# fischer-hub/panGNN

Hardware: AMD Instinct MI355X
Metric: edges/sec in GNN forward+backward (link-pred train step) (higher is better)
Workload: dtype f32

## Files before the change

### pangnn_amd/csrc/linear.hip

```cpp
#include "common.h"

namespace pangnn {

typedef float f32x16 __attribute__((ext_vector_type(16)));

__device__ __forceinline__ constexpr int jrow(int r, int hh) { return (r & 3) + 8 * (r >> 2) + 4 * hh; }

__device__ __forceinline__ void wave_sync_lds() {
  __builtin_amdgcn_fence(__ATOMIC_RELEASE, "wavefront");
  __builtin_amdgcn_wave_barrier();
  __builtin_amdgcn_fence(__ATOMIC_ACQUIRE, "wavefront");
}

__device__ __forceinline__ void pin(int64_t& base, uint32_t& off) { asm volatile("" : "+s"(base), "+v"(off)); }
__device__ __forceinline__ float4 ld_f4(const float* ubase, uint32_t byte_off) {
  typedef float f32x4 __attribute__((ext_vector_type(4)));
  const f32x4 t = __builtin_nontemporal_load(reinterpret_cast<const f32x4*>(reinterpret_cast<const char*>(ubase) + byte_off));
  return make_float4(t[0], t[1], t[2], t[3]);
}
__device__ __forceinline__ void st_f32(float* ubase, uint32_t byte_off, float v) {
  *reinterpret_cast<float*>(reinterpret_cast<char*>(ubase) + byte_off) = v;
}

typedef unsigned short bf16s;
// ... 58 lines not shown
struct RowRegs { typename Elem<T>::raw4 v[32 / (64 / (C / 4))]; };

template <int C, typename T>
__device__ __forceinline__ void load_rows_full(const T* __restrict__ src, int64_t ld, int64_t base, int lane,
                                               RowRegs<C, T>& rg) {
  constexpr int LPR = C / 4;
  constexpr int RPI = 64 / LPR;
  const int c4 = lane % LPR, r0 = lane / LPR;
  uint32_t loff = ((uint32_t)r0 * (uint32_t)ld + 4u * c4) * (uint32_t)sizeof(T);
  pin(base, loff);
#pragma unroll
  for (int i = 0; i < 32 / RPI; ++i) rg.v[i] = Elem<T>::ld4(src + (base + i * RPI) * ld, loff);
}

template <int C, typename T>
__device__ __forceinline__ void load_rows(const T* __restrict__ src, int64_t ld, int64_t n, int64_t base,
                                          int lane, RowRegs<C, T>& rg) {
  constexpr int LPR = C / 4;
  constexpr int RPI = 64 / LPR;
  const int c4 = lane % LPR, r0 = lane / LPR;
  if (base + 32 <= n) {
    load_rows_full<C, T>(src, ld, base, lane, rg);
    return;
  }
#pragma unroll
  for (int i = 0; i < 32 / RPI; ++i) {
    const int row = i * RPI + r0;
    rg.v[i] = Elem<T>::zero4();
    if (base + row < n) rg.v[i] = Elem<T>::ld4_plain(src + (base + row) * ld + 4 * c4);
  }
}

__device__ __forceinline__ float elu1(float v) { return v > 0.f ? v : __expf(v) - 1.f; }
__device__ __forceinline__ float elu1_grad(float v) { return v > 0.f ? 1.f : __expf(v); }
__device__ __forceinline__ float gen_h(float rv, float sv, float a, float c, float b) { return fmaf(rv, a, fmaf(sv, c, b)); }

template <int C, int ACT = 0, typename T = float>
__device__ __forceinline__ void store_rows(const RowRegs<C, T>& rg, int lane, float* tile) {
  constexpr int LPR = C / 4;
  constexpr int RPI = 64 / LPR;
  constexpr int RS = C + 4;
  const int c4 = lane % LPR, r0 = lane / LPR;
#pragma unroll
  for (int i = 0; i < 32 / RPI; ++i) {
    float4 v = Elem<T>::cvt4(rg.v[i]);
    if (ACT == 1) { v.x = elu1(v.x); v.y = elu1(v.y); v.z = elu1(v.z); v.w = elu1(v.w); }
    *reinterpret_cast<float4*>(tile + (i * RPI + r0) * RS + 4 * c4) = v;
  }
}

template <int K, int M>
struct FwdGeo {
  static constexpr int KS = K + 4;
  static constexpr int WAVES = (K == 128 && M == 128) ? 3 : 4;
};

template <int K, int M>
__device__ __forceinline__ void tile_product(const float* Xt, const float* Wl, int r, int hh, f32x16 (&acc)[M / 32]) {
  constexpr int KS = K + 4;
#pragma unroll
  for (int b = 0; b < M / 32; ++b)
#pragma unroll
    for (int i = 0; i < 16; ++i) acc[b][i] = 0.f;
  const float* xa = Xt + r * KS + 4 * (K / 8) * hh;
  const float* wb = Wl + r * KS + 4 * (K / 8) * hh;
  float4 a = *reinterpret_cast<const float4*>(xa);
  float4 bw[M / 32];
#pragma unroll
  for (int b = 0; b < M / 32; ++b) bw[b] = *reinterpret_cast<const float4*>(wb + 32 * b * KS);
#pragma unroll
  for (int i = 0; i < K / 8; ++i) {
    float4 an = a, bn[M / 32];
#pragma unroll
    for (int b = 0; b < M / 32; ++b) bn[b] = bw[b];
    if (i + 1 < K / 8) {
      an = *reinterpret_cast<const float4*>(xa + 4 * (i + 1));
#pragma unroll
      for (int b = 0; b < M / 32; ++b) bn[b] = *reinterpret_cast<const float4*>(wb + 32 * b * KS + 4 * (i + 1));
    }
    __builtin_amdgcn_sched_barrier(0);
#pragma unroll
    for (int b = 0; b < M / 32; ++b) {
      acc[b] = __builtin_amdgcn_mfma_f32_32x32x2f32(a.x, bw[b].x, acc[b], 0, 0, 0);
      acc[b] = __builtin_amdgcn_mfma_f32_32x32x2f32(a.y, bw[b].y, acc[b], 0, 0, 0);
      acc[b] = __builtin_amdgcn_mfma_f32_32x32x2f32(a.z, bw[b].z, acc[b], 0, 0, 0);
      acc[b] = __builtin_amdgcn_mfma_f32_32x32x2f32(a.w, bw[b].w, acc[b], 0, 0, 0);
    }
    __builtin_amdgcn_sched_barrier(0);
    a = an;
#pragma unroll
    for (int b = 0; b < M / 32; ++b) bw[b] = bn[b];
  }
}

typedef __bf16 bf16x8 __attribute__((ext_vector_type(8)));
typedef unsigned int u32x4v __attribute__((ext_vector_type(4)));
struct Split3 { bf16x8 hi, mid, lo; };
__device__ __forceinline__ Split3 split8(const float4& f0, const float4& f1) {
  const float f[8] = {f0.x, f0.y, f0.z, f0.w, f1.x, f1.y, f1.z, f1.w};
  u32x4v hi, mid, lo;
#pragma unroll
  for (int q = 0; q < 4; ++q) {
    const uint32_t a = __builtin_bit_cast(uint32_t, f[2 * q]), b = __builtin_bit_cast(uint32_t, f[2 * q + 1]);
    hi[q] = __builtin_amdgcn_perm(b, a, 0x07060302u);
    const float ra = f[2 * q] - __builtin_bit_cast(float, a & 0xffff0000u);
    const float rb = f[2 * q + 1] - __builtin_bit_cast(float, b & 0xffff0000u);
    const uint32_t ua = __builtin_bit_cast(uint32_t, ra), ub = __builtin_bit_cast(uint32_t, rb);
    mid[q] = __builtin_amdgcn_perm(ub, ua, 0x07060302u);
    const float sa = ra - __builtin_bit_cast(float, ua & 0xffff0000u);
    const float sb = rb - __builtin_bit_cast(float, ub & 0xffff0000u);
    lo[q] = __builtin_amdgcn_perm(__builtin_bit_cast(uint32_t, sb), __builtin_bit_cast(uint32_t, sa), 0x07060302u);
  }
  Split3 r;
  r.hi = __builtin_bit_cast(bf16x8, hi);
  r.mid = __builtin_bit_cast(bf16x8, mid);
  r.lo = __builtin_bit_cast(bf16x8, lo);
  return r;
}

template <int K, int M>
struct WImg {
  static constexpr int WS = K + 8;
  static constexpr bool X3 = (3 * M * WS * 2 + FwdGeo<K, M>::WAVES * 32 * (K + 4) * 4 <= 156 * 1024);
  static constexpr int FLOATS = X3 ? (3 * M * WS + 1) / 2 : M * (K + 4);
};

template <int K, int M>
__device__ __forceinline__ void stage_w(const float* __restrict__ w, int sm, int sk, float* Wl, int n_threads) {
  if constexpr (WImg<K, M>::X3) {
    constexpr int WS = WImg<K, M>::WS, IMG = M * WS;
    unsigned short* W3 = reinterpret_cast<unsigned short*>(Wl);
#pragma unroll 8
    for (int i = threadIdx.x; i < M * K; i += n_threads) {
      const int m = sk == 1 ? i / K : i % M, k = sk == 1 ? i % K : i / M;
      const float v = w[m * sm + k * sk];
      const uint32_t a = __builtin_bit_cast(uint32_t, v);
      const float r1 = v - __builtin_bit_cast(float, a & 0xffff0000u);
      const uint32_t b = __builtin_bit_cast(uint32_t, r1);
      const float r2 = r1 - __builtin_bit_cast(float, b & 0xffff0000u);
      W3[m * WS + k] = (unsigned short)(a >> 16);
      W3[IMG + m * WS + k] = (unsigned short)(b >> 16);
      W3[2 * IMG + m * WS + k] = (unsigned short)(__builtin_bit_cast(uint32_t, r2) >> 16);
    }
  } else {
    constexpr int KS = K + 4;
#pragma unroll 8
    for (int i = threadIdx.x; i < M * K; i += n_threads) {
      const int m = sk == 1 ? i / K : i % M, k = sk == 1 ? i % K : i / M;
      Wl[m * KS + k] = w[m * sm + k * sk];
    }
  }
}

template <int K, int M>
__device__ __forceinline__ void tile_product_x3(const float* Xt, const float* Wl, int r, int hh, f32x16 (&acc)[M / 32]) {
  constexpr int KS = K + 4, WS = WImg<K, M>::WS, IMG = M * WS;
#pragma unroll
  for (int b = 0; b < M / 32; ++b)
#pragma unroll
    for (int i = 0; i < 16; ++i) acc[b][i] = 0.f;
  const float* xa = Xt + r * KS + 8 * hh;
  const unsigned short* wb = reinterpret_cast<const unsigned short*>(Wl) + r * WS + 8 * hh;
  float4 x0 = *reinterpret_cast<const float4*>(xa), x1 = *reinterpret_cast<const float4*>(xa + 4);
  constexpr bool DB = (M / 32) <= 2;
  bf16x8 wf[DB ? 2 : 1][M / 32][3];
  if constexpr (DB) {
#pragma unroll
    for (int b = 0; b < M / 32; ++b)
#pragma unroll
      for (int t = 0; t < 3; ++t) wf[0][b][t] = *reinterpret_cast<const bf16x8*>(wb + 32 * b * WS + t * IMG);
  }
#pragma unroll
  for (int i = 0; i < K / 16; ++i) {
    if constexpr (!DB) {
#pragma unroll
      for (int b = 0; b < M / 32; ++b)
#pragma unroll
        for (int t = 0; t < 3; ++t) wf[0][b][t] = *reinterpret_cast<const bf16x8*>(wb + 32 * b * WS + 16 * i + t * IMG);
    }
    const Split3 a = split8(x0, x1);
    if (i + 1 < K / 16) {
      x0 = *reinterpret_cast<const float4*>(xa + 16 * (i + 1));
      x1 = *reinterpret_cast<const float4*>(xa + 16 * (i + 1) + 4);
      if constexpr (DB) {
#pragma unroll
        for (int b = 0; b < M / 32; ++b)
#pragma unroll
          for (int t = 0; t < 3; ++t)
            wf[(i + 1) & 1][b][t] = *reinterpret_cast<const bf16x8*>(wb + 32 * b * WS + 16 * (i + 1) + t * IMG);
      }
    }
#define PG_X3(AT, WT)                                                                                     \
    _Pragma("unroll") for (int b = 0; b < M / 32; ++b)                                                    \
      acc[b] = __builtin_amdgcn_mfma_f32_32x32x16_bf16(a.AT, wf[DB ? (i & 1) : 0][b][WT], acc[b], 0, 0, 0);
    PG_X3(lo, 0) PG_X3(hi, 2) PG_X3(mid, 1) PG_X3(mid, 0) PG_X3(hi, 1) PG_X3(hi, 0)
#undef PG_X3
  }
}

template <int K, int M>
__device__ __forceinline__ void tile_mult(const float* Xt, const float* Wl, int r, int hh, f32x16 (&acc)[M / 32]) {
  if constexpr (WImg<K, M>::X3) tile_product_x3<K, M>(Xt, Wl, r, hh, acc);
  else tile_product<K, M>(Xt, Wl, r, hh, acc);
}

template <int K, int M, int ACT, bool GATE, typename TX = float, typename TY = float, typename TG = float>
__global__ __launch_bounds__((FwdGeo<K, M>::WAVES * 64)) void linear_fwd_kernel(const TX* __restrict__ x, int64_t ldx,
                                                         const float* __restrict__ w, int w_sm, int w_sk,
                                                         const float* __restrict__ bias,
                                                         TY* __restrict__ y, int64_t ldy, int64_t n,
                                                         int64_t n_tiles, const TG* __restrict__ gate,
                                                         int64_t ldgate) {
  constexpr int KS = K + 4;
  constexpr int WAVES = FwdGeo<K, M>::WAVES;
  constexpr int WF = (WImg<K, M>::FLOATS + 3) & ~3;
  __shared__ __attribute__((aligned(16))) float lds[WF + WAVES * 32 * KS];
  float* Wl = lds;
  const int wave = __builtin_amdgcn_readfirstlane(threadIdx.x >> 6), lane = threadIdx.x & 63;
  float* Xt = lds + WF + wave * (32 * KS);
  stage_w<K, M>(w, w_sm, w_sk, Wl, WAVES * 64);
  __syncthreads();
  const int r = lane & 31, hh = lane >> 5;
  const int64_t stride = (int64_t)gridDim.x * WAVES;
  const int64_t n_full = n / 32;
  int64_t tile = (int64_t)blockIdx.x * WAVES + wave;
  float bv[M / 32];
#pragma unroll
  for (int b = 0; b < M / 32; ++b) bv[b] = bias ? bias[r + 32 * b] : 0.f;
  f32x16 acc[M / 32];
  RowRegs<K, TX> rg;
  if (tile < n_full) {
    const int64_t last = n_full - 1;
    load_rows_full<K, TX>(x, ldx, tile * 32, lane, rg);
    store_rows<K, ACT, TX>(rg, lane, Xt);
    load_rows_full<K, TX>(x, ldx, (tile + stride < last ? tile + stride : last) * 32, lane, rg);
    wave_sync_lds();
    for (; tile < n_full; tile += stride) {
      float gv[GATE ? M / 32 : 1][16];
      if (GATE) {
        uint32_t goff = (4u * hh * (uint32_t)ldgate + r) * (uint32_t)sizeof(TG);
        int64_t gbase = tile * 32;
        pin(gbase, goff);
#pragma unroll
        for (int i = 0; i < 16; ++i) {
          const TG* gr = gate + (gbase + (i & 3) + 8 * (i >> 2)) * ldgate;
#pragma unroll
          for (int b = 0; b < M / 32; ++b) gv[b][i] = Elem<TG>::ld1(gr + 32 * b, goff);
        }
      }
      tile_mult<K, M>(Xt, Wl, r, hh, acc);
      uint32_t loff = (4u * hh * (uint32_t)ldy + r) * (uint32_t)sizeof(TY);
      int64_t sbase = tile * 32;
      pin(sbase, loff);
#pragma unroll
      for (int i = 0; i < 16; ++i) {
        TY* yr = y + (sbase + (i & 3) + 8 * (i >> 2)) * ldy;
#pragma unroll
        for (int b = 0; b < M / 32; ++b) {
          float v = acc[b][i] + bv[b];
          if (GATE) v *= elu1_grad(gv[b][i]);
          Elem<TY>::st1(yr + 32 * b, loff, v);
        }
      }
      store_rows<K, ACT, TX>(rg, lane, Xt);
      const int64_t nxt = tile + 2 * stride;
      load_rows_full<K, TX>(x, ldx, (nxt < last ? nxt : last) * 32, lane, rg);
      wave_sync_lds();
    }
  }
  if (tile == n_full && n_full < n_tiles) {
    const int64_t base = n_full * 32;
    load_rows<K, TX>(x, ldx, n, base, lane, rg);
    wave_sync_lds();
    store_rows<K, ACT, TX>(rg, lane, Xt);
    wave_sync_lds();
    tile_mult<K, M>(Xt, Wl, r, hh, acc);
#pragma unroll
    for (int b = 0; b < M / 32; ++b)
#pragma unroll
      for (int i = 0; i < 16; ++i) {
        const int64_t row = base + jrow(i, hh);
        if (row < n) {
          float v = acc[b][i] + bv[b];
          if (GATE) v *= elu1_grad(Elem<TG>::ld1(gate + row * ldgate + r + 32 * b, 0u));
          Elem<TY>::st1(y + row * ldy + r + 32 * b, 0u, v);
        }
      }
  }
}

template <int K, int M, int ACT = 0>
__device__ __forceinline__ void wgrad_tile(const float* Xt, const float* Gt, int r, int hh, f32x16 (&acc)[M / 32][K / 32],
                                           float (&gbp)[M / 32]) {
  constexpr int KS = K + 4, MS = M + 4;
#pragma unroll
  for (int j = 0; j < 2; ++j) {
    const int row0 = 16 * j + 8 * hh;
    Split3 ga[M / 32], xb[K / 32];
#pragma unroll
    for (int a = 0; a < M / 32; ++a) {
      float f[8];
#pragma unroll
      for (int q = 0; q < 8; ++q) { f[q] = Gt[(row0 + q) * MS + r + 32 * a]; gbp[a] += f[q]; }
      ga[a] = split8(make_float4(f[0], f[1], f[2], f[3]), make_float4(f[4], f[5], f[6], f[7]));
    }
#pragma unroll
    for (int b = 0; b < K / 32; ++b) {
      float f[8];
#pragma unroll
      for (int q = 0; q < 8; ++q) {
        f[q] = Xt[(row0 + q) * KS + r + 32 * b];
        if (ACT == 1) f[q] = elu1(f[q]);
      }
      xb[b] = split8(make_float4(f[0], f[1], f[2], f[3]), make_float4(f[4], f[5], f[6], f[7]));
    }
#define PG_W3(GT, XT)                                                                                     \
    _Pragma("unroll") for (int a = 0; a < M / 32; ++a)                                                    \
    _Pragma("unroll") for (int b = 0; b < K / 32; ++b)                                                    \
      acc[a][b] = __builtin_amdgcn_mfma_f32_32x32x16_bf16(ga[a].GT, xb[b].XT, acc[a][b], 0, 0, 0);
    PG_W3(lo, hi) PG_W3(hi, lo) PG_W3(mid, mid) PG_W3(mid, hi) PG_W3(hi, mid) PG_W3(hi, hi)
#undef PG_W3
  }
}

template <int K, int M>
__device__ __forceinline__ void gen_wgrad_tile_x3(const float* Gt, const float* rs, const float (&ca)[K / 32],
                                                  const float (&cc)[K / 32], const float (&cb)[K / 32], int r, int hh,
                                                  f32x16 (&acc)[M / 32][K / 32], float (&gbp)[M / 32]) {
  constexpr int MS = M + 4;
#pragma unroll
  for (int j = 0; j < 2; ++j) {
    const int row0 = 16 * j + 8 * hh;
    const float4 R0 = *reinterpret_cast<const float4*>(rs + row0), R1 = *reinterpret_cast<const float4*>(rs + row0 + 4);
    const float4 S0 = *reinterpret_cast<const float4*>(rs + 32 + row0), S1 = *reinterpret_cast<const float4*>(rs + 32 + row0 + 4);
    const float rr[8] = {R0.x, R0.y, R0.z, R0.w, R1.x, R1.y, R1.z, R1.w};
    const float ss[8] = {S0.x, S0.y, S0.z, S0.w, S1.x, S1.y, S1.z, S1.w};
    Split3 ga[M / 32], xb[K / 32];
#pragma unroll
    for (int a = 0; a < M / 32; ++a) {
      float f[8];
#pragma unroll
      for (int q = 0; q < 8; ++q) { f[q] = Gt[(row0 + q) * MS + r + 32 * a]; gbp[a] += f[q]; }
      ga[a] = split8(make_float4(f[0], f[1], f[2], f[3]), make_float4(f[4], f[5], f[6], f[7]));
    }
#pragma unroll
    for (int b = 0; b < K / 32; ++b) {
      float f[8];
#pragma unroll
      for (int q = 0; q < 8; ++q) f[q] = elu1(gen_h(rr[q], ss[q], ca[b], cc[b], cb[b]));
      xb[b] = split8(make_float4(f[0], f[1], f[2], f[3]), make_float4(f[4], f[5], f[6], f[7]));
    }
#define PG_W3(GT, XT)                                                                                     \
    _Pragma("unroll") for (int a = 0; a < M / 32; ++a)                                                    \
    _Pragma("unroll") for (int b = 0; b < K / 32; ++b)                                                    \
      acc[a][b] = __builtin_amdgcn_mfma_f32_32x32x16_bf16(ga[a].GT, xb[b].XT, acc[a][b], 0, 0, 0);
    PG_W3(lo, hi) PG_W3(hi, lo) PG_W3(mid, mid) PG_W3(mid, hi) PG_W3(hi, mid) PG_W3(hi, hi)
#undef PG_W3
  }
}

template <int K, int M>
struct WgradGeo {
  static constexpr int SLAB = M * K + M;
};

template <int K, int M, int LDS_F>
__device__ __forceinline__ void wgrad_finish(const f32x16 (&acc)[M / 32][K / 32], const float (&gbp)[M / 32], float* lds,
                                             float* __restrict__ slab, int wave, int lane) {
  constexpr int NA = (M / 32) * (K / 32) * 16, NV = NA + M / 32;
  static_assert(2 * NV * 64 <= LDS_F, "tree buffers of the wgrad finish");
  const int r = lane & 31, hh = lane >> 5;
  float val[NV];
#pragma unroll
  for (int a = 0; a < M / 32; ++a) {
#pragma unroll
    for (int b = 0; b < K / 32; ++b)
#pragma unroll
      for (int i = 0; i < 16; ++i) val[(a * (K / 32) + b) * 16 + i] = acc[a][b][i];
    val[NA + a] = gbp[a];
  }
  __syncthreads();
#pragma unroll
  for (int d = 1; d < 4; d <<= 1) {
    const bool writer = (wave & (2 * d - 1)) == d, reader = (wave & (2 * d - 1)) == 0;
    float* mine = lds + (size_t)(d == 1 ? (wave >> 1) : 0) * (NV * 64) + lane;
    if (writer) {
#pragma unroll
      for (int v = 0; v < NV; ++v) mine[v * 64] = val[v];
    }
    __syncthreads();
    if (reader) {
#pragma unroll
      for (int v = 0; v < NV; ++v) val[v] += mine[v * 64];
    }
    __syncthreads();
  }
  if (wave == 0) {
#pragma unroll
    for (int a = 0; a < M / 32; ++a) {
#pragma unroll
      for (int b = 0; b < K / 32; ++b)
#pragma unroll
        for (int i = 0; i < 16; ++i) lds[(32 * a + jrow(i, hh)) * K + r + 32 * b] = val[(a * (K / 32) + b) * 16 + i];
      if (hh == 0) lds[M * K + r + 32 * a] = val[NA + a];
    }
  }
  __syncthreads();
  for (int i = threadIdx.x; i < M * K + M; i += 256) slab[i] = lds[i];
}

template <int K, int M, int ACT, typename TG = float, typename TX = float>
__global__ __launch_bounds__(256) void linear_wgrad_kernel(const TG* __restrict__ g, int64_t ldg,
                                                           const TX* __restrict__ x, int64_t ldx,
                                                           int64_t n, int64_t n_tiles,
                                                           float* __restrict__ slabs) {
  constexpr int KS = K + 4, MS = M + 4;
  constexpr int PER_WAVE = 32 * KS + 32 * MS;
  constexpr int SLAB = WgradGeo<K, M>::SLAB;
  constexpr int LDS_F = (4 * PER_WAVE > SLAB) ? 4 * PER_WAVE : SLAB;
  __shared__ __attribute__((aligned(16))) float lds[LDS_F];
  const int wave = __builtin_amdgcn_readfirstlane(threadIdx.x >> 6), lane = threadIdx.x & 63;
  float* Xt = lds + wave * PER_WAVE;
  float* Gt = Xt + 32 * KS;
  const int r = lane & 31, hh = lane >> 5;
  f32x16 acc[M / 32][K / 32];
  float gbp[M / 32];
#pragma unroll
  for (int a = 0; a < M / 32; ++a) {
    gbp[a] = 0.f;
#pragma unroll
    for (int b = 0; b < K / 32; ++b)
#pragma unroll
      for (int i = 0; i < 16; ++i) acc[a][b][i] = 0.f;
  }
  const int64_t stride = (int64_t)gridDim.x * 4;
  int64_t tile = (int64_t)blockIdx.x * 4 + wave;
  RowRegs<K, TX> rx;
  RowRegs<M, TG> rgm;
  load_rows<K, TX>(x, ldx, n, tile * 32, lane, rx);
  load_rows<M, TG>(g, ldg, n, tile * 32, lane, rgm);
  for (; tile < n_tiles; tile += stride) {
    store_rows<K, ACT, TX>(rx, lane, Xt);
    store_rows<M, 0, TG>(rgm, lane, Gt);
    load_rows<K, TX>(x, ldx, n, (tile + stride) * 32, lane, rx);
    load_rows<M, TG>(g, ldg, n, (tile + stride) * 32, lane, rgm);
    wave_sync_lds();
    wgrad_tile<K, M>(Xt, Gt, r, hh, acc, gbp);
    wave_sync_lds();
  }
#pragma unroll
  for (int a = 0; a < M / 32; ++a) gbp[a] += __shfl_xor(gbp[a], 32);
  wgrad_finish<K, M, LDS_F>(acc, gbp, lds, slabs + (int64_t)blockIdx.x * SLAB, wave, lane);
}

__global__ __launch_bounds__(kSumThreads) void slab_reduce_kernel(const float* __restrict__ slabs, int n_slabs,
                                                                  int slab_len, int split,
                                                                  float* __restrict__ out0,
                                                                  float* __restrict__ out1) {
  const int i = blockIdx.x * kWave + (threadIdx.x & (kWave - 1));
  const float s = ordered_parts_sum(slabs, n_slabs, slab_len, i, slab_len);
  if (threadIdx.x >= kWave || i >= slab_len) return;
  if (i < split) out0[i] = s;
  else if (out1) out1[i - split] = s;
}

static int num_cus() {
  int dev = 0, v = 0;
  if (hipGetDevice(&dev) == hipSuccess &&
      hipDeviceGetAttribute(&v, hipDeviceAttributeMultiprocessorCount, dev) == hipSuccess && v > 0)
    return v;
  return 256;
}

template <int K, int M, typename TX, typename TY, typename TG>
static int launch_fwd_t(const void* x, int64_t ldx, const float* w, int w_trans, const float* bias, void* y, int64_t ldy,
                        int64_t n, int in_act, const void* gate, int64_t ldgate, hipStream_t s) {
  const int w_sm = w_trans ? 1 : K, w_sk = w_trans ? M : 1;
  constexpr int WAVES = FwdGeo<K, M>::WAVES;
  const int64_t n_tiles = (n + 31) / 32;
  int64_t grid = (n_tiles + WAVES - 1) / WAVES;
  const int64_t cap = (int64_t)num_cus();
  if (grid > cap) grid = cap;
  const dim3 g((unsigned)grid), b(WAVES * 64);
  const TX* xp = static_cast<const TX*>(x);
  TY* yp = static_cast<TY*>(y);
  const TG* gp = static_cast<const TG*>(gate);
  if (gate)
    hipLaunchKernelGGL((linear_fwd_kernel<K, M, 0, true, TX, TY, TG>), g, b, 0, s, xp, ldx, w, w_sm, w_sk, bias, yp, ldy, n, n_tiles, gp, ldgate);
  else if (in_act)
    hipLaunchKernelGGL((linear_fwd_kernel<K, M, 1, false, TX, TY, float>), g, b, 0, s, xp, ldx, w, w_sm, w_sk, bias, yp, ldy, n, n_tiles,
                       static_cast<const float*>(nullptr), ldgate);
  else
    hipLaunchKernelGGL((linear_fwd_kernel<K, M, 0, false, TX, TY, float>), g, b, 0, s, xp, ldx, w, w_sm, w_sk, bias, yp, ldy, n, n_tiles,
                       static_cast<const float*>(nullptr), ldgate);
  PG_CHECK_LAUNCH("pangnn_linear_fwd");
  return 0;
}

template <int K, int M, typename H>
static int launch_fwd(const void* x, int x16, int64_t ldx, const float* w, int w_trans, const float* bias, void* y,
                      int y16, int64_t ldy, int64_t n, int in_act, const void* gate, int gate16, int64_t ldgate,
                      hipStream_t s) {
#define PG_FWD(TX, TY, TG) return launch_fwd_t<K, M, TX, TY, TG>(x, ldx, w, w_trans, bias, y, ldy, n, in_act, gate, ldgate, s)
  if (gate) {
    if (gate16) { if (x16) PG_FWD(H, H, H); PG_FWD(float, H, H); }
    if (x16) PG_FWD(H, float, float);
    PG_FWD(float, float, float);
  }
  if (x16) { if (y16) PG_FWD(H, H, float); PG_FWD(H, float, float); }
  if (y16) PG_FWD(float, H, float);
// ... 394 lines not shown
      x0.z = elu1(gen_h(rv, sv, a0.z, c0.z, b0.z)); x0.w = elu1(gen_h(rv, sv, a0.w, c0.w, b0.w));
      x1.x = elu1(gen_h(rv, sv, a1.x, c1.x, b1.x)); x1.y = elu1(gen_h(rv, sv, a1.y, c1.y, b1.y));
      x1.z = elu1(gen_h(rv, sv, a1.z, c1.z, b1.z)); x1.w = elu1(gen_h(rv, sv, a1.w, c1.w, b1.w));
      const Split3 a = split8(x0, x1);
#define PG_X3(AT, WT)                                                                                     \
      _Pragma("unroll") for (int b = 0; b < M / 32; ++b)                                                  \
        acc[b] = __builtin_amdgcn_mfma_f32_32x32x16_bf16(a.AT, wf[b][WT], acc[b], 0, 0, 0);
      PG_X3(lo, 0) PG_X3(hi, 2) PG_X3(mid, 1) PG_X3(mid, 0) PG_X3(hi, 1) PG_X3(hi, 0)
#undef PG_X3
    }
    if (tile * 32 + 32 <= n) {
      uint32_t loff = (4u * hh * (uint32_t)ldy + r) * (uint32_t)sizeof(float);
      int64_t sbase = tile * 32;
      pin(sbase, loff);
#pragma unroll
      for (int i = 0; i < 16; ++i) {
        float* yr = y + (sbase + (i & 3) + 8 * (i >> 2)) * ldy;
#pragma unroll
        for (int b = 0; b < M / 32; ++b) st_f32(yr + 32 * b, loff, acc[b][i] + bv[b]);
      }
    } else {
#pragma unroll
      for (int b = 0; b < M / 32; ++b)
#pragma unroll
        for (int i = 0; i < 16; ++i) {
          const int64_t row = tile * 32 + jrow(i, hh);
          if (row < n) y[row * ldy + r + 32 * b] = acc[b][i] + bv[b];
        }
    }
    rv = rn;
    sv = sn;
  }
}

template <int K, int M>
__global__ __launch_bounds__(256) void gen_linear_wgrad_kernel(const float* __restrict__ g, int64_t ldg,
                                                               const float* __restrict__ rvec, const float* __restrict__ svec,
                                                               const float* __restrict__ w_emb, const float* __restrict__ b_emb,
                                                               const float* __restrict__ w_in, const float* __restrict__ b_in,
                                                               int D, int64_t n, int64_t n_tiles, float* __restrict__ slabs) {
  constexpr int KS = K + 4, MS = M + 4;
  constexpr int PER_WAVE = 32 * KS + 32 * MS;
  constexpr int SLAB = WgradGeo<K, M>::SLAB;
  constexpr int LDS_F = (4 * PER_WAVE > SLAB) ? 4 * PER_WAVE : SLAB;
  __shared__ __attribute__((aligned(16))) float lds[LDS_F];
  __shared__ __attribute__((aligned(16))) float acb[3 * K];
  const int wave = __builtin_amdgcn_readfirstlane(threadIdx.x >> 6), lane = threadIdx.x & 63;
  float* Xt = lds + wave * PER_WAVE;
  float* Gt = Xt + 32 * KS;
  gen_params<K>(w_emb, b_emb, w_in, b_in, D, acb, 256);
  __syncthreads();
  const int r = lane & 31, hh = lane >> 5;
  float ca[K / 32], cc[K / 32], cb[K / 32];
#pragma unroll
  for (int b = 0; b < K / 32; ++b) { ca[b] = acb[r + 32 * b]; cc[b] = acb[K + r + 32 * b]; cb[b] = acb[2 * K + r + 32 * b]; }
  f32x16 acc[M / 32][K / 32];
  float gbp[M / 32];
#pragma unroll
  for (int a = 0; a < M / 32; ++a) {
    gbp[a] = 0.f;
#pragma unroll
    for (int b = 0; b < K / 32; ++b)
#pragma unroll
      for (int i = 0; i < 16; ++i) acc[a][b][i] = 0.f;
  }
  const int64_t stride = (int64_t)gridDim.x * 4;
  int64_t tile = (int64_t)blockIdx.x * 4 + wave;
  RowRegs<M, float> rgm;
  float rsv = gen_load(rvec, svec, n, tile * 32, lane);
  load_rows<M, float>(g, ldg, n, tile * 32, lane, rgm);
  for (; tile < n_tiles; tile += stride) {
    Xt[lane] = rsv;
    store_rows<M, 0, float>(rgm, lane, Gt);
    rsv = gen_load(rvec, svec, n, (tile + stride) * 32, lane);
    load_rows<M, float>(g, ldg, n, (tile + stride) * 32, lane, rgm);
    wave_sync_lds();
    gen_wgrad_tile_x3<K, M>(Gt, Xt, ca, cc, cb, r, hh, acc, gbp);
    wave_sync_lds();
  }
#pragma unroll
  for (int a = 0; a < M / 32; ++a) gbp[a] += __shfl_xor(gbp[a], 32);
  wgrad_finish<K, M, LDS_F>(acc, gbp, lds, slabs + (int64_t)blockIdx.x * SLAB, wave, lane);
}

template <int KG, int H>
__global__ __launch_bounds__((FwdGeo<KG, H>::WAVES * 64)) void gen_linear_dgrad_sums_kernel(
    const float* __restrict__ g, int64_t ldg, const float* __restrict__ w_out, const float* __restrict__ rvec,
    const float* __restrict__ svec, const float* __restrict__ w_emb, const float* __restrict__ b_emb,
    const float* __restrict__ w_in, const float* __restrict__ b_in, int D, int64_t n, int64_t n_tiles,
    float* __restrict__ slabs) {
  constexpr int KS = KG + 4;
  constexpr int WAVES = FwdGeo<KG, H>::WAVES;
  constexpr int WF = (WImg<KG, H>::FLOATS + 3) & ~3;
  __shared__ __attribute__((aligned(16))) float lds[WF + WAVES * 32 * KS];
  __shared__ __attribute__((aligned(16))) float acb[3 * H];
  __shared__ float part[WAVES][3 * H];
  float* Wl = lds;
  const int wave = __builtin_amdgcn_readfirstlane(threadIdx.x >> 6), lane = threadIdx.x & 63;
  float* Xt = lds + WF + wave * (32 * KS);
  stage_w<KG, H>(w_out, 1, H, Wl, WAVES * 64);
  gen_params<H>(w_emb, b_emb, w_in, b_in, D, acb, WAVES * 64);
  __syncthreads();
  const int r = lane & 31, hh = lane >> 5;
  float ca[H / 32], cc[H / 32], cb[H / 32];
#pragma unroll
  for (int b = 0; b < H / 32; ++b) { ca[b] = acb[r + 32 * b]; cc[b] = acb[H + r + 32 * b]; cb[b] = acb[2 * H + r + 32 * b]; }
  float s0[H / 32], s1[H / 32], s2[H / 32];
#pragma unroll
  for (int b = 0; b < H / 32; ++b) s0[b] = s1[b] = s2[b] = 0.f;
  const int64_t stride = (int64_t)gridDim.x * WAVES;
  int64_t tile = (int64_t)blockIdx.x * WAVES + wave;
  f32x16 acc[H / 32];
  RowRegs<KG, float> rg;
  load_rows<KG, float>(g, ldg, n, tile * 32, lane, rg);
  float rsv = gen_load(rvec, svec, n, tile * 32, lane);
  for (; tile < n_tiles; tile += stride) {
    store_rows<KG, 0, float>(rg, lane, Xt);
    const float rs_cur = rsv;
    load_rows<KG, float>(g, ldg, n, (tile + stride) * 32, lane, rg);
    rsv = gen_load(rvec, svec, n, (tile + stride) * 32, lane);
    wave_sync_lds();
    tile_mult<KG, H>(Xt, Wl, r, hh, acc);
#pragma unroll
    for (int i = 0; i < 16; ++i) {
      const int row = jrow(i, hh);
      const float rv = __shfl(rs_cur, row), sv = __shfl(rs_cur, 32 + row);
#pragma unroll
      for (int b = 0; b < H / 32; ++b) {
        const float v = acc[b][i] * elu1_grad(gen_h(rv, sv, ca[b], cc[b], cb[b]));
        s0[b] = fmaf(rv, v, s0[b]);
        s1[b] = fmaf(sv, v, s1[b]);
        s2[b] += v;
      }
    }
    wave_sync_lds();
  }
#pragma unroll
  for (int b = 0; b < H / 32; ++b) {
    s0[b] += __shfl_xor(s0[b], 32);
    s1[b] += __shfl_xor(s1[b], 32);
    s2[b] += __shfl_xor(s2[b], 32);
    if (hh == 0) { part[wave][r + 32 * b] = s0[b]; part[wave][H + r + 32 * b] = s1[b]; part[wave][2 * H + r + 32 * b] = s2[b]; }
  }
  __syncthreads();
  float* slab = slabs + (int64_t)blockIdx.x * (3 * H);
  for (int i = threadIdx.x; i < 3 * H; i += WAVES * 64) {
    float t = part[0][i];
#pragma unroll
    for (int wv = 1; wv < WAVES; ++wv) t += part[wv][i];
    slab[i] = t;
  }
}

template <int K, int M>
static int launch_gen_fwd(const float* r, const float* sv, const float* w_emb, const float* b_emb, const float* w_in,
                          const float* b_in, int D, const float* w, const float* bias, float* y, int64_t ldy, int64_t n,
                          hipStream_t s) {
  const int64_t n_tiles = (n + 31) / 32;
  if constexpr (WImg<K, M>::X3) {
    int64_t grid = (n_tiles + 7) / 8;
    const int64_t cap = 2 * (int64_t)num_cus();
    if (grid > cap) grid = cap;
    hipLaunchKernelGGL((gen_linear_fwd_reg_kernel<K, M>), dim3((unsigned)grid), dim3(512), 0, s, r, sv, w_emb, b_emb, w_in, b_in,
                       D, w, bias, y, ldy, n, n_tiles);
    PG_CHECK_LAUNCH("pangnn_embed_linear_fwd");
    return 0;
  }
  constexpr int WAVES = FwdGeo<K, M>::WAVES;
  int64_t grid = (n_tiles + WAVES - 1) / WAVES;
  const int64_t cap = (int64_t)num_cus();
  if (grid > cap) grid = cap;
  hipLaunchKernelGGL((gen_linear_fwd_kernel<K, M>), dim3((unsigned)grid), dim3(WAVES * 64), 0, s, r, sv, w_emb, b_emb, w_in, b_in,
                     D, w, bias, y, ldy, n, n_tiles);
  PG_CHECK_LAUNCH("pangnn_embed_linear_fwd");
  return 0;
}

static int64_t gen_grid(int64_t n, int waves) {
  const int64_t n_tiles = (n + 31) / 32;
  int64_t grid = (n_tiles + waves - 1) / waves;
  const int64_t cap = (int64_t)num_cus();
  if (grid > cap) grid = cap;
  return grid < 1 ? 1 : grid;
}

template <int K, int M>
static int launch_gen_bwd(const float* g, int64_t ldg, const float* r, const float* sv, const float* w_emb, const float* b_emb,
                          const float* w_in, const float* b_in, int D, const float* w_out, int64_t n, float* g_w_out,
                          float* g_b_out, float* sums, float* ws, hipStream_t s) {
  constexpr int SLAB = WgradGeo<K, M>::SLAB;
  const int64_t n_tiles = (n + 31) / 32;
  const int64_t grid_w = gen_grid(n, 4);
  hipLaunchKernelGGL((gen_linear_wgrad_kernel<K, M>), dim3((unsigned)grid_w), dim3(256), 0, s, g, ldg, r, sv, w_emb, b_emb, w_in,
                     b_in, D, n, n_tiles, ws);
  PG_CHECK_LAUNCH("pangnn_embed_linear_bwd(wgrad)");
  hipLaunchKernelGGL(slab_reduce_kernel, dim3((SLAB + kWave - 1) / kWave), dim3(kSumThreads), 0, s, ws, (int)grid_w, SLAB,
                     M * K, g_w_out, g_b_out);
  PG_CHECK_LAUNCH("pangnn_embed_linear_bwd(wgrad reduce)");
  float* ws2 = ws + (size_t)num_cus() * SLAB;
  constexpr int WAVES = FwdGeo<M, K>::WAVES;
  const int64_t grid_d = gen_grid(n, WAVES);
  hipLaunchKernelGGL((gen_linear_dgrad_sums_kernel<M, K>), dim3((unsigned)grid_d), dim3(WAVES * 64), 0, s, g, ldg, w_out, r, sv,
                     w_emb, b_emb, w_in, b_in, D, n, n_tiles, ws2);
  PG_CHECK_LAUNCH("pangnn_embed_linear_bwd(dgrad sums)");
  hipLaunchKernelGGL(slab_reduce_kernel, dim3((3 * K + kWave - 1) / kWave), dim3(kSumThreads), 0, s, ws2, (int)grid_d, 3 * K,
                     3 * K, sums, static_cast<float*>(nullptr));
  PG_CHECK_LAUNCH("pangnn_embed_linear_bwd(sums reduce)");
  return 0;
}

}

using namespace pangnn;

extern "C" int pangnn_linear_supported(int32_t K, int32_t M, int wgrad) {
  const bool km = (K == 64 || K == 128) && (M == 64 || M == 128);
  if (!km) return 0;
  (void)wgrad;
  return 1;
}

static bool dtype_ok(int32_t d) { return d == PANGNN_DTYPE_F32 || d == PANGNN_DTYPE_BF16 || d == PANGNN_DTYPE_F16; }
static int fmt16_of(int32_t a, int32_t b, int32_t c = PANGNN_DTYPE_F32) {
  int f = 0;
  for (int32_t d : {a, b, c}) {
    if (d == PANGNN_DTYPE_F32) continue;
    if (f && f != d) return -1;
    f = d;
  }
  return f;
}
static bool aligned8(const void* p) { return (reinterpret_cast<uintptr_t>(p) & 7u) == 0; }

static int linear_fwd_common(const void* x, int32_t x_dtype, int64_t ldx, const float* w, int w_trans, const float* bias,
                             void* y, int32_t y_dtype, int64_t ldy, int64_t n, int32_t K, int32_t M, int32_t in_act,
                             const void* gate, int32_t gate_dtype, int64_t ldgate, pangnn_stream_t stream) {
  PG_CHECK_ARG(n >= 0, PANGNN_E_BADARG, "pangnn_linear_fwd: negative size");
  PG_CHECK_ARG(pangnn_linear_supported(K, M, 0), PANGNN_E_BADARG,
               "pangnn_linear_fwd: K and M must be 64 or 128 (got %d, %d)", (int)K, (int)M);
  PG_CHECK_ARG(dtype_ok(x_dtype) && dtype_ok(y_dtype) && (!gate || dtype_ok(gate_dtype)), PANGNN_E_BADARG,
               "pangnn_linear_fwd: storage types are PANGNN_DTYPE_F32 / _BF16 / _F16");
  PG_CHECK_ARG((in_act == 0 || in_act == 1) && !(in_act && gate) && (!gate || ldgate >= M), PANGNN_E_BADARG,
               "pangnn_linear_act_fwd: in_act must be 0 or 1 (ELU) and excludes gate; ldgate >= M");
  PG_CHECK_ARG(!gate || gate_dtype == y_dtype, PANGNN_E_BADARG,
               "pangnn_linear_act_fwd: a gated product is stored like its gate (it is the gate tensor's gradient)");
  if (n == 0) return 0;
  PG_CHECK_ARG(x && w && y && ldx >= K && ldy >= M, PANGNN_E_BADARG, "pangnn_linear_fwd: bad pointer / ld");
  PG_CHECK_ARG((x_dtype != PANGNN_DTYPE_F32 ? aligned8(x) : aligned16(x)) && aligned16(w) && ldx % 4 == 0,
               PANGNN_E_ALIGN, "pangnn_linear_fwd: x rows must start on 16 bytes (f32) / 8 bytes (bf16, f16), w on 16, ldx % 4 == 0");
  const int fmt = fmt16_of(x_dtype, y_dtype, gate ? gate_dtype : PANGNN_DTYPE_F32);
  PG_CHECK_ARG(fmt >= 0, PANGNN_E_BADARG, "pangnn_linear_fwd: the 2-byte operands of one call are all bfloat16 or all float16");
  hipStream_t s = (hipStream_t)stream;
  const int xb = x_dtype != PANGNN_DTYPE_F32, yb = y_dtype != PANGNN_DTYPE_F32, gb = gate && gate_dtype != PANGNN_DTYPE_F32;
#define PG_SHAPES(H)                                                                                                              \
  do {                                                                                                                            \
    if (K == 64 && M == 64) return launch_fwd<64, 64, H>(x, xb, ldx, w, w_trans, bias, y, yb, ldy, n, in_act, gate, gb, ldgate, s);   \
    if (K == 64 && M == 128) return launch_fwd<64, 128, H>(x, xb, ldx, w, w_trans, bias, y, yb, ldy, n, in_act, gate, gb, ldgate, s); \
    if (K == 128 && M == 64) return launch_fwd<128, 64, H>(x, xb, ldx, w, w_trans, bias, y, yb, ldy, n, in_act, gate, gb, ldgate, s); \
    return launch_fwd<128, 128, H>(x, xb, ldx, w, w_trans, bias, y, yb, ldy, n, in_act, gate, gb, ldgate, s);                         \
  } while (0)
  if (fmt == PANGNN_DTYPE_F16) PG_SHAPES(f16s);
  PG_SHAPES(bf16s);
#undef PG_SHAPES
}

extern "C" int pangnn_linear_act_fwd_mixed(const void* x, int32_t x_dtype, int64_t ldx, const float* w, const float* bias,
                                           void* y, int32_t y_dtype, int64_t ldy, int64_t n, int32_t K, int32_t M,
                                           int32_t in_act, const void* gate, int32_t gate_dtype, int64_t ldgate,
                                           pangnn_stream_t stream) {
  return linear_fwd_common(x, x_dtype, ldx, w, 0, bias, y, y_dtype, ldy, n, K, M, in_act, gate, gate_dtype, ldgate, stream);
}

extern "C" int pangnn_linear_dgrad_mixed(const void* g, int32_t g_dtype, int64_t ldg, const float* w, void* gx,
                                         int32_t gx_dtype, int64_t ldgx, int64_t n, int32_t K, int32_t M, const void* gate,
                                         int32_t gate_dtype, int64_t ldgate, pangnn_stream_t stream) {
  return linear_fwd_common(g, g_dtype, ldg, w, 1, nullptr, gx, gx_dtype, ldgx, n, M, K, 0, gate, gate_dtype, ldgate, stream);
}

extern "C" int pangnn_linear_act_fwd_f32(const float* x, int64_t ldx, const float* w, const float* bias, float* y,
                                         int64_t ldy, int64_t n, int32_t K, int32_t M, int32_t in_act,
                                         const float* gate, int64_t ldgate, pangnn_stream_t stream) {
  return pangnn_linear_act_fwd_mixed(x, PANGNN_DTYPE_F32, ldx, w, bias, y, PANGNN_DTYPE_F32, ldy, n, K, M, in_act, gate,
                                     PANGNN_DTYPE_F32, ldgate, stream);
}

extern "C" int pangnn_linear_fwd_f32(const float* x, int64_t ldx, const float* w, const float* bias, float* y,
                                     int64_t ldy, int64_t n, int32_t K, int32_t M, pangnn_stream_t stream) {
  return pangnn_linear_act_fwd_f32(x, ldx, w, bias, y, ldy, n, K, M, 0, nullptr, 0, stream);
}

extern "C" size_t pangnn_linear_wgrad_workspace_bytes(int32_t K, int32_t M) {
  return (size_t)num_cus() * ((size_t)M * K + M) * sizeof(float);
}

extern "C" int pangnn_linear_act_wgrad_mixed(const void* g, int32_t g_dtype, int64_t ldg, const void* x, int32_t x_dtype,
                                             int64_t ldx, int64_t n, int32_t K, int32_t M, int32_t in_act, float* gw,
                                             float* gb, void* workspace, size_t workspace_bytes, pangnn_stream_t stream) {
  PG_CHECK_ARG(n >= 0, PANGNN_E_BADARG, "pangnn_linear_wgrad: negative size");
  PG_CHECK_ARG(pangnn_linear_supported(K, M, 1), PANGNN_E_BADARG,
               "pangnn_linear_wgrad: unsupported (K, M) = (%d, %d)", (int)K, (int)M);
  PG_CHECK_ARG(in_act == 0 || in_act == 1, PANGNN_E_BADARG, "pangnn_linear_act_wgrad: in_act must be 0 or 1");
  PG_CHECK_ARG(dtype_ok(g_dtype) && dtype_ok(x_dtype), PANGNN_E_BADARG,
               "pangnn_linear_wgrad: storage types are PANGNN_DTYPE_F32 / _BF16 / _F16");
  PG_CHECK_ARG(gw && (n == 0 || (g && x)) && ldg >= M && ldx >= K, PANGNN_E_BADARG,
               "pangnn_linear_wgrad: bad pointer / ld");
  PG_CHECK_ARG((g_dtype != PANGNN_DTYPE_F32 ? aligned8(g) : aligned16(g)) &&
                   (x_dtype != PANGNN_DTYPE_F32 ? aligned8(x) : aligned16(x)) && ldg % 4 == 0 && ldx % 4 == 0,
               PANGNN_E_ALIGN, "pangnn_linear_wgrad: rows must start on 16 bytes (f32) / 8 bytes (bf16, f16), ld multiples of 4");
  const int fmt = fmt16_of(g_dtype, x_dtype);
  PG_CHECK_ARG(fmt >= 0, PANGNN_E_BADARG, "pangnn_linear_wgrad: the 2-byte operands of one call are all bfloat16 or all float16");
  hipStream_t s = (hipStream_t)stream;
  float* ws = static_cast<float*>(workspace);
  const int gbf = g_dtype != PANGNN_DTYPE_F32, xbf = x_dtype != PANGNN_DTYPE_F32;
#define PG_SHAPES(H)                                                                                                                 \
  do {                                                                                                                               \
    if (K == 64 && M == 64) return launch_wgrad<64, 64, H>(g, gbf, ldg, x, xbf, ldx, n, in_act, gw, gb, ws, workspace_bytes, s);      \
    if (K == 64 && M == 128) return launch_wgrad<64, 128, H>(g, gbf, ldg, x, xbf, ldx, n, in_act, gw, gb, ws, workspace_bytes, s);    \
    if (K == 128 && M == 128) {                                                                                                      \
        \
                              \
      const char* g_hi = static_cast<const char*>(g) + (size_t)64 * (gbf ? 2 : 4);                                                   \
      int rc = launch_wgrad<128, 64, H>(g, gbf, ldg, x, xbf, ldx, n, in_act, gw, gb, ws, workspace_bytes, s);                         \
      if (rc) return rc;                                                                                                             \
      return launch_wgrad<128, 64, H>(g_hi, gbf, ldg, x, xbf, ldx, n, in_act, gw + (size_t)64 * 128, gb ? gb + 64 : nullptr, ws,      \
                                      workspace_bytes, s);                                                                           \
    }                                                                                                                                \
    return launch_wgrad<128, 64, H>(g, gbf, ldg, x, xbf, ldx, n, in_act, gw, gb, ws, workspace_bytes, s);                             \
  } while (0)
  if (fmt == PANGNN_DTYPE_F16) PG_SHAPES(f16s);
  PG_SHAPES(bf16s);
#undef PG_SHAPES
}

extern "C" int pangnn_linear_act_wgrad_f32(const float* g, int64_t ldg, const float* x, int64_t ldx, int64_t n,
                                           int32_t K, int32_t M, int32_t in_act, float* gw, float* gb,
                                           void* workspace, size_t workspace_bytes, pangnn_stream_t stream) {
  return pangnn_linear_act_wgrad_mixed(g, PANGNN_DTYPE_F32, ldg, x, PANGNN_DTYPE_F32, ldx, n, K, M, in_act, gw, gb,
                                       workspace, workspace_bytes, stream);
}

extern "C" int pangnn_linear_wgrad_f32(const float* g, int64_t ldg, const float* x, int64_t ldx, int64_t n,
                                       int32_t K, int32_t M, float* gw, float* gb, void* workspace,
                                       size_t workspace_bytes, pangnn_stream_t stream) {
  return pangnn_linear_act_wgrad_f32(g, ldg, x, ldx, n, K, M, 0, gw, gb, workspace, workspace_bytes, stream);
}
// ... 74 lines not shown
```

Baseline: 6.555 billion.

## Fuse embed-linear wgrad and dgrad-sums into one warp-specialized backward kernel

For the K=128, M=64 case, the separate wgrad and dgrad-sums kernels are replaced by one 512-thread kernel. Four waves load G and r/s tiles into double-buffered LDS and compute the dgrad sums, while the other four waves consume the same tiles for the weight gradient. This removes one kernel launch and avoids reading G and the embedding inputs from global memory twice. In exchange it adds barrier coupling between the two roles and a dummy-barrier count that must match wgrad_finish. The dgrad path is split into 2-block halves, with rounding arranged to keep results identical, and an environment variable can turn the fused path off.

```diff
diff --git a/pangnn_amd/csrc/linear.hip b/pangnn_amd/csrc/linear.hip
--- a/pangnn_amd/csrc/linear.hip
+++ b/pangnn_amd/csrc/linear.hip
@@ -234,21 +234,20 @@
   }
 }
 
-template <int K, int M>
-__device__ __forceinline__ void tile_product_x3(const float* Xt, const float* Wl, int r, int hh, f32x16 (&acc)[M / 32]) {
+template <int K, int M, int NB, int B0, bool DB = (NB <= 2)>
+__device__ __forceinline__ void tile_product_x3_blocks(const float* Xt, const float* Wl, int r, int hh, f32x16 (&acc)[NB]) {
   constexpr int KS = K + 4, WS = WImg<K, M>::WS, IMG = M * WS;
 #pragma unroll
-  for (int b = 0; b < M / 32; ++b)
+  for (int b = 0; b < NB; ++b)
 #pragma unroll
     for (int i = 0; i < 16; ++i) acc[b][i] = 0.f;
   const float* xa = Xt + r * KS + 8 * hh;
-  const unsigned short* wb = reinterpret_cast<const unsigned short*>(Wl) + r * WS + 8 * hh;
+  const unsigned short* wb = reinterpret_cast<const unsigned short*>(Wl) + (r + 32 * B0) * WS + 8 * hh;
   float4 x0 = *reinterpret_cast<const float4*>(xa), x1 = *reinterpret_cast<const float4*>(xa + 4);
-  constexpr bool DB = (M / 32) <= 2;
-  bf16x8 wf[DB ? 2 : 1][M / 32][3];
+  bf16x8 wf[DB ? 2 : 1][NB][3];
   if constexpr (DB) {
 #pragma unroll
-    for (int b = 0; b < M / 32; ++b)
+    for (int b = 0; b < NB; ++b)
 #pragma unroll
       for (int t = 0; t < 3; ++t) wf[0][b][t] = *reinterpret_cast<const bf16x8*>(wb + 32 * b * WS + t * IMG);
   }
@@ -256,7 +255,7 @@
   for (int i = 0; i < K / 16; ++i) {
     if constexpr (!DB) {
 #pragma unroll
-      for (int b = 0; b < M / 32; ++b)
+      for (int b = 0; b < NB; ++b)
 #pragma unroll
         for (int t = 0; t < 3; ++t) wf[0][b][t] = *reinterpret_cast<const bf16x8*>(wb + 32 * b * WS + 16 * i + t * IMG);
     }
@@ -266,18 +265,23 @@
       x1 = *reinterpret_cast<const float4*>(xa + 16 * (i + 1) + 4);
       if constexpr (DB) {
 #pragma unroll
-        for (int b = 0; b < M / 32; ++b)
+        for (int b = 0; b < NB; ++b)
 #pragma unroll
           for (int t = 0; t < 3; ++t)
             wf[(i + 1) & 1][b][t] = *reinterpret_cast<const bf16x8*>(wb + 32 * b * WS + 16 * (i + 1) + t * IMG);
       }
     }
 #define PG_X3(AT, WT)                                                                                     \
-    _Pragma("unroll") for (int b = 0; b < M / 32; ++b)                                                    \
+    _Pragma("unroll") for (int b = 0; b < NB; ++b)                                                        \
       acc[b] = __builtin_amdgcn_mfma_f32_32x32x16_bf16(a.AT, wf[DB ? (i & 1) : 0][b][WT], acc[b], 0, 0, 0);
     PG_X3(lo, 0) PG_X3(hi, 2) PG_X3(mid, 1) PG_X3(mid, 0) PG_X3(hi, 1) PG_X3(hi, 0)
 #undef PG_X3
   }
+}
+
+template <int K, int M>
+__device__ __forceinline__ void tile_product_x3(const float* Xt, const float* Wl, int r, int hh, f32x16 (&acc)[M / 32]) {
+  tile_product_x3_blocks<K, M, M / 32, 0>(Xt, Wl, r, hh, acc);
 }
 
 template <int K, int M>
@@ -438,6 +442,42 @@
       acc[a][b] = __builtin_amdgcn_mfma_f32_32x32x16_bf16(ga[a].GT, xb[b].XT, acc[a][b], 0, 0, 0);
     PG_W3(lo, hi) PG_W3(hi, lo) PG_W3(mid, mid) PG_W3(mid, hi) PG_W3(hi, mid) PG_W3(hi, hi)
 #undef PG_W3
+  }
+}
+
+template <int K, int M>
+__device__ __forceinline__ void gen_wgrad_tile_x3_by_block(const float* Gt, const float* rs, const float* acb, int r, int hh,
+                                                           f32x16 (&acc)[M / 32][K / 32], float (&gbp)[M / 32]) {
+  constexpr int MS = M + 4;
+#pragma unroll
+  for (int j = 0; j < 2; ++j) {
+    const int row0 = 16 * j + 8 * hh;
+    Split3 ga[M / 32];
+#pragma unroll
+    for (int a = 0; a < M / 32; ++a) {
+      float f[8];
+#pragma unroll
+      for (int q = 0; q < 8; ++q) { f[q] = Gt[(row0 + q) * MS + r + 32 * a]; gbp[a] += f[q]; }
+      ga[a] = split8(make_float4(f[0], f[1], f[2], f[3]), make_float4(f[4], f[5], f[6], f[7]));
+    }
+#pragma unroll
+    for (int b = 0; b < K / 32; ++b) {
+      const float4 R0 = *reinterpret_cast<const float4*>(rs + row0), R1 = *reinterpret_cast<const float4*>(rs + row0 + 4);
+      const float4 S0 = *reinterpret_cast<const float4*>(rs + 32 + row0), S1 = *reinterpret_cast<const float4*>(rs + 32 + row0 + 4);
+      const float rr[8] = {R0.x, R0.y, R0.z, R0.w, R1.x, R1.y, R1.z, R1.w};
+      const float ss[8] = {S0.x, S0.y, S0.z, S0.w, S1.x, S1.y, S1.z, S1.w};
+      const float ca = acb[r + 32 * b], cc = acb[K + r + 32 * b], cb = acb[2 * K + r + 32 * b];
+      float f[8];
+#pragma unroll
+      for (int q = 0; q < 8; ++q) f[q] = elu1(gen_h(rr[q], ss[q], ca, cc, cb));
+      const Split3 xb = split8(make_float4(f[0], f[1], f[2], f[3]), make_float4(f[4], f[5], f[6], f[7]));
+#define PG_W3(GT, XT)                                                                                     \
+      _Pragma("unroll") for (int a = 0; a < M / 32; ++a)                                                  \
+        acc[a][b] = __builtin_amdgcn_mfma_f32_32x32x16_bf16(ga[a].GT, xb.XT, acc[a][b], 0, 0, 0);
+      PG_W3(lo, hi) PG_W3(hi, lo) PG_W3(mid, mid) PG_W3(mid, hi) PG_W3(hi, mid) PG_W3(hi, hi)
+#undef PG_W3
+      __builtin_amdgcn_sched_barrier(0);
+    }
   }
 }
 
@@ -1138,6 +1178,130 @@
   }
 }
 
+constexpr int kWgradFinishBarriers = 6;
+
+__device__ __forceinline__ float add_rounded(float a, float b) {
+#pragma clang fp contract(off)
+  return a + b;
+}
+
+template <int H, int M>
+__global__ __launch_bounds__(512) void gen_linear_bwd_pairs_kernel(
+    const float* __restrict__ g, int64_t ldg, const float* __restrict__ w_out, const float* __restrict__ rvec,
+    const float* __restrict__ svec, const float* __restrict__ w_emb, const float* __restrict__ b_emb,
+    const float* __restrict__ w_in, const float* __restrict__ b_in, int D, int64_t n, int64_t n_tiles,
+    float* __restrict__ slabs_w, float* __restrict__ slabs_s) {
+  static_assert(M == 64 && H == 128 && WImg<M, H>::X3 && FwdGeo<M, H>::WAVES == 4, "the two kernels' common geometry");
+  constexpr int MS = M + 4;
+  constexpr int TILE = 32 * MS + 64;
+  constexpr int WF = (WImg<M, H>::FLOATS + 3) & ~3;
+  constexpr int TILES_F = 2 * 4 * TILE;
+  constexpr int SLAB = WgradGeo<H, M>::SLAB;
+  static_assert(TILES_F >= SLAB, "slab image of the wgrad finish");
+  __shared__ __attribute__((aligned(16))) float lds[WF + TILES_F];
+  __shared__ __attribute__((aligned(16))) float acb[3 * H];
+  __shared__ float part[4][3 * H];
+  float* Wl = lds;
+  float* tiles = lds + WF;
+  const int wave = __builtin_amdgcn_readfirstlane(threadIdx.x >> 6), lane = threadIdx.x & 63;
+  const int role = wave >> 2, pair = wave & 3;
+  stage_w<M, H>(w_out, 1, H, Wl, 512);
+  gen_params<H>(w_emb, b_emb, w_in, b_in, D, acb, 512);
+  __syncthreads();
+  const int r = lane & 31, hh = lane >> 5;
+  const int64_t stride = (int64_t)gridDim.x * 4, first = (int64_t)blockIdx.x * 4;
+  const int rounds = first < n_tiles ? (int)((n_tiles - first + stride - 1) / stride) : 0;
+  int64_t tile = first + pair;
+  if (role == 0) {
+    f32x16 acc[M / 32][H / 32];
+    float gbp[M / 32];
+#pragma unroll
+    for (int a = 0; a < M / 32; ++a) {
+      gbp[a] = 0.f;
+#pragma unroll
+      for (int b = 0; b < H / 32; ++b)
+#pragma unroll
+        for (int i = 0; i < 16; ++i) acc[a][b][i] = 0.f;
+    }
+    for (int k = 0; k < rounds; ++k, tile += stride) {
+      const float* Gt = tiles + ((k & 1) * 4 + pair) * TILE;
+      __syncthreads();
+      if (tile < n_tiles) gen_wgrad_tile_x3_by_block<H, M>(Gt, Gt + 32 * MS, acb, r, hh, acc, gbp);
+    }
+#pragma unroll
+    for (int a = 0; a < M / 32; ++a) gbp[a] += __shfl_xor(gbp[a], 32);
+    wgrad_finish<H, M, TILES_F>(acc, gbp, tiles, slabs_w + (int64_t)blockIdx.x * SLAB, pair, lane);
+  } else {
+    float s0[H / 32], s1[H / 32], s2[H / 32];
+#pragma unroll
+    for (int b = 0; b < H / 32; ++b) s0[b] = s1[b] = s2[b] = 0.f;
+    RowRegs<M, float> rg;
+    load_rows<M, float>(g, ldg, n, tile * 32, lane, rg);
+    float rsv = gen_load(rvec, svec, n, tile * 32, lane);
+    for (int k = 0; k < rounds; ++k, tile += stride) {
+      float* Gt = tiles + ((k & 1) * 4 + pair) * TILE;
+      store_rows<M, 0, float>(rg, lane, Gt);
+      Gt[32 * MS + lane] = rsv;
+      load_rows<M, float>(g, ldg, n, (tile + stride) * 32, lane, rg);
+      rsv = gen_load(rvec, svec, n, (tile + stride) * 32, lane);
+      __syncthreads();
+      if (tile < n_tiles) {
+        const float* rs = Gt + 32 * MS;
+#pragma unroll
+        for (int hb = 0; hb < H / 32; hb += 2) {
+          if (hb) __builtin_amdgcn_sched_barrier(0);
+          f32x16 acc[2];
+          if (hb == 0) tile_product_x3_blocks<M, H, 2, 0, false>(Gt, Wl, r, hh, acc);
+          else tile_product_x3_blocks<M, H, 2, 2, false>(Gt, Wl, r, hh, acc);
+          float ca[2], cc[2], cb[2];
+#pragma unroll
+          for (int b = 0; b < 2; ++b) {
+            ca[b] = acb[r + 32 * (hb + b)];
+            cc[b] = acb[H + r + 32 * (hb + b)];
+            cb[b] = acb[2 * H + r + 32 * (hb + b)];
+          }
+#pragma unroll
+          for (int i4 = 0; i4 < 4; ++i4) {
+            const float4 R = *reinterpret_cast<const float4*>(rs + 8 * i4 + 4 * hh);
+            const float4 S = *reinterpret_cast<const float4*>(rs + 32 + 8 * i4 + 4 * hh);
+            const float rq[4] = {R.x, R.y, R.z, R.w}, sq[4] = {S.x, S.y, S.z, S.w};
+#pragma unroll
+            for (int q = 0; q < 4; ++q) {
+              const float rv = rq[q], sv = sq[q];
+#pragma unroll
+              for (int b = 0; b < 2; ++b) {
+                const float e = elu1_grad(gen_h(rv, sv, ca[b], cc[b], cb[b]));
+                const float v = acc[b][4 * i4 + q] * e;
+                s0[hb + b] = fmaf(rv, v, s0[hb + b]);
+                s1[hb + b] = fmaf(sv, v, s1[hb + b]);
+                if (hb == 0 || i4 == 0) s2[hb + b] = fmaf(acc[b][4 * i4 + q], e, s2[hb + b]);
+                else s2[hb + b] = add_rounded(s2[hb + b], v);
+              }
+            }
+          }
+        }
+      }
+    }
+#pragma unroll
+    for (int b = 0; b < H / 32; ++b) {
+      s0[b] += __shfl_xor(s0[b], 32);
+      s1[b] += __shfl_xor(s1[b], 32);
+      s2[b] += __shfl_xor(s2[b], 32);
+      if (hh == 0) { part[pair][r + 32 * b] = s0[b]; part[pair][H + r + 32 * b] = s1[b]; part[pair][2 * H + r + 32 * b] = s2[b]; }
+    }
+    __syncthreads();
+    float* slab = slabs_s + (int64_t)blockIdx.x * (3 * H);
+    for (int i = threadIdx.x - 256; i < 3 * H; i += 256) {
+      float t = part[0][i];
+#pragma unroll
+      for (int wv = 1; wv < 4; ++wv) t += part[wv][i];
+      slab[i] = t;
+    }
+#pragma unroll
+    for (int i = 1; i < kWgradFinishBarriers; ++i) __syncthreads();
+  }
+}
+
 template <int K, int M>
 static int launch_gen_fwd(const float* r, const float* sv, const float* w_emb, const float* b_emb, const float* w_in,
                           const float* b_in, int D, const float* w, const float* bias, float* y, int64_t ldy, int64_t n,
@@ -1177,6 +1341,22 @@
   constexpr int SLAB = WgradGeo<K, M>::SLAB;
   const int64_t n_tiles = (n + 31) / 32;
   const int64_t grid_w = gen_grid(n, 4);
+  if constexpr (K == 128 && M == 64) {
+    const char* one = getenv("PANGNN_GEN_BWD_ONE_LAUNCH");
+    if (!(one && one[0] == '0' && one[1] == 0)) {
+      float* ws_s = ws + (size_t)num_cus() * SLAB;
+      hipLaunchKernelGGL((gen_linear_bwd_pairs_kernel<K, M>), dim3((unsigned)grid_w), dim3(512), 0, s, g, ldg, w_out, r, sv, w_emb,
+                         b_emb, w_in, b_in, D, n, n_tiles, ws, ws_s);
+      PG_CHECK_LAUNCH("pangnn_embed_linear_bwd(pairs)");
+      hipLaunchKernelGGL(slab_reduce_kernel, dim3((SLAB + kWave - 1) / kWave), dim3(kSumThreads), 0, s, ws, (int)grid_w, SLAB,
+                         M * K, g_w_out, g_b_out);
+      PG_CHECK_LAUNCH("pangnn_embed_linear_bwd(wgrad reduce)");
+      hipLaunchKernelGGL(slab_reduce_kernel, dim3((3 * K + kWave - 1) / kWave), dim3(kSumThreads), 0, s, ws_s, (int)grid_w, 3 * K,
+                         3 * K, sums, static_cast<float*>(nullptr));
+      PG_CHECK_LAUNCH("pangnn_embed_linear_bwd(sums reduce)");
+      return 0;
+    }
+  }
   hipLaunchKernelGGL((gen_linear_wgrad_kernel<K, M>), dim3((unsigned)grid_w), dim3(256), 0, s, g, ldg, r, sv, w_emb, b_emb, w_in,
                      b_in, D, n, n_tiles, ws);
   PG_CHECK_LAUNCH("pangnn_embed_linear_bwd(wgrad)");
```

Result: no change. 6.565 billion (median of 6 runs) (+0.2%).
